# OVGULIU/cedar

Measured on AMD Instinct MI355X. Metric: fine-grid DOF/s per V-cycle, higher is better.
Workload: dtype f64; 1 GPU; 3D 27-pt gallery::fe Poisson-type, 512^3, 8-colour GS V(2,1); levels=8, cycle=V(2,1), relaxation=point, parallelism=single GPU

## Files before the change

cedar_amd/csrc/relax27_dev.h:

```cpp
#pragma once
#include "common.h"

namespace cedar_amd {

struct C27 {
	real_t pw, ps, psw, b, bw, bs, bsw;
	real_t pnw_n, ps_n, bnw_n, bn_n;
	real_t b_t, be_t, bn_t, bne_t;
	real_t bse_nt, bs_nt;
	real_t psw_ne, bne_ne;
	real_t pw_e, pnw_e, be_e, bse_e;
	real_t bsw_net;
	real_t bw_et, bnw_et;
};

__device__ __forceinline__ real_t offdiag27(real_t qf, const C27 &c, const real_t (&qq)[3][3][3])
{
	real_t s = qf;
	s = s + c.pw * qq[1][1][0];
	s = s + c.pnw_n * qq[1][2][0];
	s = s + c.ps_n * qq[1][2][1];
	s = s + c.psw_ne * qq[1][2][2];
	s = s + c.pw_e * qq[1][1][2];
	s = s + c.pnw_e * qq[1][0][2];
	s = s + c.ps * qq[1][0][1];
	s = s + c.psw * qq[1][0][0];
	s = s + c.b * qq[0][1][1];
	s = s + c.bw * qq[0][1][0];
	s = s + c.bnw_n * qq[0][2][0];
	s = s + c.bn_n * qq[0][2][1];
	s = s + c.bne_ne * qq[0][2][2];
	s = s + c.be_e * qq[0][1][2];
	s = s + c.bse_e * qq[0][0][2];
	s = s + c.bs * qq[0][0][1];
	s = s + c.bsw * qq[0][0][0];
	s = s + c.b_t * qq[2][1][1];
	s = s + c.be_t * qq[2][1][0];
	s = s + c.bse_nt * qq[2][2][0];
	s = s + c.bs_nt * qq[2][2][1];
	s = s + c.bsw_net * qq[2][2][2];
	s = s + c.bw_et * qq[2][1][2];
	s = s + c.bnw_et * qq[2][0][2];
	s = s + c.bn_t * qq[2][0][1];
	s = s + c.bne_t * qq[2][0][0];
	return s;
}


__device__ __forceinline__ void ldpair(const real_t *__restrict__ p, bool two, real_t &a, real_t &b)
{
	if (two) {
		d2u v = *reinterpret_cast<const d2u *>(p);
		a = v.x; b = v.y;
	} else {
		a = p[0]; b = 0.0;
	}
}

__device__ __forceinline__ void ldpair(const float *__restrict__ p, bool two, real_t &a, real_t &b)
{
	if (two) {
		f2u v = *reinterpret_cast<const f2u *>(p);
		a = (real_t)v.x; b = (real_t)v.y;
	} else {
		a = (real_t)p[0]; b = 0.0;
	}
}

template <bool NT>
__device__ __forceinline__ void ldpair_so(const real_t *__restrict__ p, bool two, real_t &a, real_t &b)
{
	if (!NT) { ldpair(p, two, a, b); return; }
	if (two) {
		d2u v = __builtin_nontemporal_load(reinterpret_cast<const d2u *>(p));
		a = v.x; b = v.y;
	} else {
		a = __builtin_nontemporal_load(p); b = 0.0;
	}
}

template <bool NT>
__device__ __forceinline__ void ldpair_so(const float *__restrict__ p, bool two, real_t &a, real_t &b)
{
	if (!NT) { ldpair(p, two, a, b); return; }
	if (two) {
		f2u v = __builtin_nontemporal_load(reinterpret_cast<const f2u *>(p));
		a = (real_t)v.x; b = (real_t)v.y;
	} else {
		a = (real_t)__builtin_nontemporal_load(p); b = 0.0;
	}
}

#define WI_SLOT(slot) ((size_t)(((WI & 4) && ((slot) == KB || (slot) >= KBW)) ? KPW : (slot)))
template <bool NT, bool NTP = NT, bool NTO = NT, int WI = 0, typename OP = Op3>
__device__ __forceinline__ void load_coef27(const OP &A, size_t rowA, int ie, int io, bool two, C27 &ce, C27 &co)
{
	const auto *__restrict__ so = A.so;
	const size_t PS = A.SS, aj = A.SJ, ak = (WI & 2) ? 0 : A.SK;
#define LD_I_(N, slot, off, fe, fo)                                                    \
{                                                                                  \
	real_t a_, b_;                                                                 \
	ldpair_so<N>(so + WI_SLOT(slot)*PS + rowA + (off) + ie, true, a_, b_);         \
	ce.fe = a_; co.fo = b_;                                                        \
}
#define LD_I(slot, off, fe, fo) LD_I_(NT, slot, off, fe, fo)
#define LD_IO(slot, fe, fo) LD_I_(NTO, slot, 0, fe, fo)
#define LD_IS(slot, off, fe, fo) LD_I_(NTP, slot, off, fe, fo)
#define LD_ISO(slot, fe, fo) LD_I_((NTP && NTO), slot, 0, fe, fo)
	LD_IO(KPW, pw, pw) LD_ISO(KPS, ps, ps) LD_ISO(KPSW, psw, psw) LD_IO(KB, b, b)
	LD_IO(KBW, bw, bw) LD_IO(KBS, bs, bs) LD_IO(KBSW, bsw, bsw)
	LD_IS(KPNW, aj, pnw_n, pnw_n) LD_IS(KPS, aj, ps_n, ps_n) LD_I(KBNW, aj, bnw_n, bnw_n) LD_I(KBN, aj, bn_n, bn_n)
	LD_I(KB, ak, b_t, b_t) LD_I(KBE, ak, be_t, be_t) LD_I(KBN, ak, bn_t, bn_t) LD_I(KBNE, ak, bne_t, bne_t)
	LD_I(KBSE, aj + ak, bse_nt, bse_nt) LD_I(KBS, aj + ak, bs_nt, bs_nt)
#undef LD_I
#undef LD_IO
#undef LD_IS
#undef LD_ISO
#undef LD_I_
#define LD_IP_(N, slot, off, f)                                                        \
{                                                                                  \
	real_t a_, b_;                                                                 \
	ldpair_so<N>(so + WI_SLOT(slot)*PS + rowA + (off) + io, two, a_, b_);          \
	ce.f = a_; co.f = b_;                                                          \
}
#define LD_IP(slot, off, f) LD_IP_(NT, slot, off, f)
#define LD_IPO(slot, f) LD_IP_(NTO, slot, 0, f)
#define LD_IPS(slot, off, f) LD_IP_(NTP, slot, off, f)
#define LD_IPSO(slot, f) LD_IP_((NTP && NTO), slot, 0, f)
	LD_IPS(KPSW, aj, psw_ne) LD_IP(KBNE, aj, bne_ne)
	LD_IPO(KPW, pw_e) LD_IPSO(KPNW, pnw_e) LD_IPO(KBE, be_e) LD_IPO(KBSE, bse_e)
	LD_IP(KBSW, aj + ak, bsw_net)
	LD_IP(KBW, ak, bw_et) LD_IP(KBNW, ak, bnw_et)
#undef LD_IP
#undef LD_IPO
#undef LD_IPS
#undef LD_IPSO
#undef LD_IP_
}

template <int WI = 0>
__device__ __forceinline__ void load_vec27(const real_t *__restrict__ qf, const real_t *__restrict__ q, size_t row, size_t sj,
                                           size_t sk, int ie, int io, bool two,
                                           real_t (&qe)[3][3][3], real_t (&qo)[3][3][3], real_t &qfe, real_t &qfo)
{
	if (WI & 1) { sj = 0; sk = 0; }
	{
		real_t a_, b_;
		ldpair(qf + row + ie, true, a_, b_); qfe = a_; qfo = b_;
	}
#pragma unroll
	for (int dk = 0; dk < 3; dk++)
#pragma unroll
		for (int dj = 0; dj < 3; dj++) {
			const real_t *r = q + row + (ptrdiff_t)(dj - 1) * (ptrdiff_t)sj + (ptrdiff_t)(dk - 1) * (ptrdiff_t)sk;
			real_t w0, w1, w2, w3;
			ldpair(r + ie - 1, true, w0, w1);
			ldpair(r + io, two, w2, w3);
			qe[dk][dj][0] = w0; qe[dk][dj][1] = w1; qe[dk][dj][2] = w2;
			qo[dk][dj][0] = w1; qo[dk][dj][1] = w2; qo[dk][dj][2] = w3;
		}
}

template <bool NT, bool NTP = NT, bool NTO = NT, int WI = 0, typename OP = Op3>
__device__ __forceinline__ void load_pair27(const OP &A, const real_t *__restrict__ qf,
                                            const real_t *__restrict__ q, size_t rowA, size_t row, size_t sj, size_t sk,
                                            int ie, int io, bool two, C27 &ce, C27 &co,
                                            real_t (&qe)[3][3][3], real_t (&qo)[3][3][3], real_t &qfe, real_t &qfo)
{
	load_coef27<NT, NTP, NTO, WI>(A, rowA, ie, io, two, ce, co);
	load_vec27<WI>(qf, q, row, sj, sk, ie, io, two, qe, qo, qfe, qfo);
}

__device__ __forceinline__ void skip27_lane(unsigned skm, int p, int P, bool &ske, bool &sko)
{
	if (skm & 0x100u) { ske = sko = true; return; }
	const int slot = p == 0 ? 0 : p == 1 ? 2 : p == P - 2 ? 4 : p == P - 1 ? 6 : -1;
	ske = slot >= 0 && ((skm >> slot) & 1u);
	sko = slot >= 0 && ((skm >> (slot + 1)) & 1u);
}

template <int BS, bool EFIRST, bool NT, bool NTP = NT, int WI = 0, bool PERX = false, bool MSK = false, typename OP = Op3>
__device__ __forceinline__ void relax27_row_task(const OP &A, const real_t *__restrict__ qf,
                                                 real_t *__restrict__ q, int II, size_t sj, size_t sk,
                                                 size_t j, size_t k, real_t *xch, unsigned skm = 0)
{
	const size_t row = j * sj + k * sk, rowA = j * A.SJ + k * A.SK;
	const int p = threadIdx.x;
	const int ie = 2 * p + 1, io = 2 * p + 2;
	const bool e_ok = ie <= II - 2;
	const bool o_ok = io <= II - 2;
	const bool two = io + 1 <= II - 1;

	real_t e_new = 0.0, o_new = 0.0;
	C27 ce, co;
	real_t qe[3][3][3], qo[3][3][3];
	real_t qfe = 0, qfo = 0, sre = 0, sro = 0;

	if (e_ok) {
		load_pair27<NT, NTP, NT, WI>(A, qf, q, rowA, row, sj, sk, ie, io, two, ce, co, qe, qo, qfe, qfo);
		real_t a_, b_;
		ldpair(A.sor + j * A.rSJ + k * A.rSK + ie, true, a_, b_); sre = a_; sro = b_;
	}

	bool ske = false, sko = false;
	if (MSK) skip27_lane(skm, p, (II - 2 + 1) / 2, ske, sko);
	if (EFIRST) {
		if (e_ok) {
			e_new = (MSK && ske) ? qe[1][1][1] : offdiag27(qfe, ce, qe) * sre;
			xch[p] = e_new;
		}
		__syncthreads();
		if (o_ok) {
			qo[1][1][0] = e_new;
			if (io + 1 <= II - 2) qo[1][1][2] = xch[p + 1];
			else if (PERX) qo[1][1][2] = xch[0];
			o_new = (MSK && sko) ? qo[1][1][1] : offdiag27(qfo, co, qo) * sro;
		}
		if (PERX && o_ok && io == II - 2) {
			q[row] = o_new;
			q[row + II - 1] = xch[0];
		}
	} else {
		if (o_ok) {
			o_new = (MSK && sko) ? qo[1][1][1] : offdiag27(qfo, co, qo) * sro;
			xch[p + 1] = o_new;
		}
		__syncthreads();
		if (e_ok) {
			if (p > 0) qe[1][1][0] = xch[p];
			else if (PERX) qe[1][1][0] = xch[(II - 2) / 2];
			if (o_ok) qe[1][1][2] = o_new;
			e_new = (MSK && ske) ? qe[1][1][1] : offdiag27(qfe, ce, qe) * sre;
		}
		if (PERX && p == 0 && e_ok) {
			q[row] = xch[(II - 2) / 2];
			q[row + II - 1] = e_new;
		}
	}
	if (e_ok) {
		if (o_ok) {
			d2u v; v.x = e_new; v.y = o_new;
			*reinterpret_cast<d2u *>(q + row + ie) = v;
		} else {
			q[row + ie] = e_new;
		}
	}
}

}
```

cedar_amd/csrc/relax3d_psum.hip:

```cpp
#include "common.h"
#include "relax27_dev.h"
#include "relax3_psum.h"
#include <vector>

namespace cedar_amd {

struct PsumGeom { int jbF, frun, nF, nS, nrun; };

__host__ __device__ static inline PsumGeom psum_geom(int JJ, int jbF, int frun)
{
	PsumGeom g;
	g.jbF = jbF; g.frun = frun;
	g.nF = (JJ - 2 - jbF + 1) / 2;
	g.nS = (JJ - 2 - (1 - jbF) + 1) / 2;
	g.nrun = (g.nF + frun - 1) / frun;
	return g;
}

__host__ __device__ static inline void psum_run_range(const PsumGeom &g, int JJ, int run, int &lo, int &hi)
{
	const int f0 = run * g.frun, f1 = (f0 + g.frun < g.nF) ? f0 + g.frun : g.nF;
	lo = 1 + g.jbF + 2 * f0;
	hi = 1 + g.jbF + 2 * (f1 - 1);
	if (g.jbF && f0 == 0) lo = 1;
	if (f1 == g.nF && hi + 1 <= JJ - 2) hi = hi + 1;
}

__host__ __device__ static inline bool psum_row_ok(const PsumGeom &g, int JJ, int j)
{
	int f = (j - 1 - g.jbF) >> 1;
	if (f < 0) f = 0;
	if (f >= g.nF) f = g.nF - 1;
	int lo, hi;
	psum_run_range(g, JJ, f / g.frun, lo, hi);
	return lo + 1 <= j && j <= hi - 1;
}

__host__ __device__ static inline bool psum_a_gives(int k, int KK, int nbr)
{
	return k >= 1 && k <= KK - 2 && !(k == 1 && (nbr & 1)) && !(k == KK - 2 && (nbr & 2));
}
__host__ __device__ static inline bool psum_b_takes(int kp, int KK, int nbr)
{
	return kp - 1 >= 1 && kp + 1 <= KK - 2 && psum_a_gives(kp - 1, KK, nbr) && psum_a_gives(kp + 1, KK, nbr);
}

template <int SIDE, int DI, int DJ>
__device__ __forceinline__ real_t kcoef(const C27 &c)
{
	if (SIDE == 0) {
		if (DI == 0 && DJ == 0) return c.b_t;
		if (DI == -1 && DJ == 0) return c.be_t;
		if (DI == -1 && DJ == 1) return c.bse_nt;
		if (DI == 0 && DJ == 1) return c.bs_nt;
		if (DI == 1 && DJ == 1) return c.bsw_net;
		if (DI == 1 && DJ == 0) return c.bw_et;
		if (DI == 1 && DJ == -1) return c.bnw_et;
		if (DI == 0 && DJ == -1) return c.bn_t;
		return c.bne_t;
	}
	if (DI == 0 && DJ == 0) return c.b;
	if (DI == -1 && DJ == 0) return c.bw;
	if (DI == -1 && DJ == 1) return c.bnw_n;
	if (DI == 0 && DJ == 1) return c.bn_n;
	if (DI == 1 && DJ == 1) return c.bne_ne;
	if (DI == 1 && DJ == 0) return c.be_e;
	if (DI == 1 && DJ == -1) return c.bse_e;
	if (DI == 0 && DJ == -1) return c.bs;
	return c.bsw;
}

template <int BS>
struct PsumLds {
	real_t xch[2][BS + 2];
	real_t exP[6][BS + 1];
	real_t exN[6][BS + 1];
	real_t acc[4][2][2 * BS];
};

template <int BS, bool EFIRST, bool NT, typename OP = Op3>
__device__ __forceinline__ void relax27_row_task_A(const OP &A, const real_t *__restrict__ qf, real_t *__restrict__ q,
                                                   real_t *__restrict__ T, int II, size_t sj, size_t sk, size_t j, size_t k,
                                                   PsumLds<BS> &S, int t, bool isf, int lo, int hi, bool stU, bool stD,
                                                   unsigned skm)
{
	const size_t row = j * sj + k * sk, rowA = j * A.SJ + k * A.SK;
	const int p = threadIdx.x;
	const int ie = 2 * p + 1, io = 2 * p + 2;
	const bool e_ok = ie <= II - 2;
	const bool o_ok = io <= II - 2;
	const bool two = io + 1 <= II - 1;
	real_t *xch = S.xch[t & 1];

	real_t e_new = 0.0, o_new = 0.0;
	C27 ce, co;
	real_t qe[3][3][3], qo[3][3][3];
	real_t qfe = 0, qfo = 0, sre = 0, sro = 0;

	if (e_ok) {
		load_pair27<NT, false, NT, 0>(A, qf, q, rowA, row, sj, sk, ie, io, two, ce, co, qe, qo, qfe, qfo);
		real_t a_, b_;
		ldpair(A.sor + j * A.rSJ + k * A.rSK + ie, true, a_, b_); sre = a_; sro = b_;
	}
	const real_t ghostL = qe[1][1][0];
	const real_t ghostR = o_ok ? qo[1][1][2] : qe[1][1][2];

	bool ske = false, sko = false;
	if (skm) skip27_lane(skm, p, (II - 2 + 1) / 2, ske, sko);
	if (EFIRST) {
		if (e_ok) {
			e_new = ske ? qe[1][1][1] : offdiag27(qfe, ce, qe) * sre;
			xch[p] = e_new;
		}
		__syncthreads();
		if (o_ok) {
			qo[1][1][0] = e_new;
			if (io + 1 <= II - 2) qo[1][1][2] = xch[p + 1];
			o_new = sko ? qo[1][1][1] : offdiag27(qfo, co, qo) * sro;
		}
	} else {
		if (o_ok) {
			o_new = sko ? qo[1][1][1] : offdiag27(qfo, co, qo) * sro;
			xch[p + 1] = o_new;
		}
		__syncthreads();
		if (e_ok) {
			if (p > 0) qe[1][1][0] = xch[p];
			if (o_ok) qe[1][1][2] = o_new;
			e_new = ske ? qe[1][1][1] : offdiag27(qfe, ce, qe) * sre;
		}
	}
	if (e_ok) {
		if (o_ok) {
			d2u v; v.x = e_new; v.y = o_new;
			*reinterpret_cast<d2u *>(q + row + ie) = v;
		} else {
			q[row + ie] = e_new;
		}
	}
	if (!stU && !stD) return;

	const real_t se = e_new, so_ = o_ok ? o_new : ghostR;
	const bool last_o = o_ok && io == II - 2;
	real_t own_e[6], own_o[6];
	const auto *__restrict__ sop = A.so;
	const size_t PS = A.SS, aj = A.SJ, ak = A.SK;
	if (e_ok) {
#define GROUP(SIDE, DJ)                                                                                           \
	{                                                                                                             \
		constexpr int g_ = SIDE * 3 + (DJ + 1);                                                                   \
		own_e[g_] = se * kcoef<SIDE, 0, DJ>(ce);                                                                  \
		if (o_ok || io == II - 1) own_e[g_] = own_e[g_] + so_ * kcoef<SIDE, -1, DJ>(co);                          \
		S.exP[g_][p] = se * kcoef<SIDE, -1, DJ>(ce);                                                              \
		if (o_ok) {                                                                                               \
			own_o[g_] = se * kcoef<SIDE, 1, DJ>(ce) + so_ * kcoef<SIDE, 0, DJ>(co);                               \
			S.exN[g_][p + 1] = so_ * kcoef<SIDE, 1, DJ>(co);                                                      \
		}                                                                                                         \
	}
		GROUP(0, -1) GROUP(0, 0) GROUP(0, 1) GROUP(1, -1) GROUP(1, 0) GROUP(1, 1)
#undef GROUP
		if (p == 0) {
			S.exN[0][0] = ghostL * sop[KBNW * PS + rowA + ak + 1];
			S.exN[1][0] = ghostL * sop[KBW * PS + rowA + ak + 1];
			S.exN[2][0] = ghostL * sop[KBSW * PS + rowA + aj + ak + 1];
			S.exN[3][0] = ghostL * sop[KBSE * PS + rowA + 1];
			S.exN[4][0] = ghostL * sop[KBE * PS + rowA + 1];
			S.exN[5][0] = ghostL * sop[KBNE * PS + rowA + aj + 1];
		}
		if (last_o) {
			const size_t x = (size_t)(II - 1);
			S.exP[0][p + 1] = ghostR * sop[KBNE * PS + rowA + ak + x];
			S.exP[1][p + 1] = ghostR * sop[KBE * PS + rowA + ak + x];
			S.exP[2][p + 1] = ghostR * sop[KBSE * PS + rowA + aj + ak + x];
			S.exP[3][p + 1] = ghostR * sop[KBSW * PS + rowA + x];
			S.exP[4][p + 1] = ghostR * sop[KBW * PS + rowA + x];
			S.exP[5][p + 1] = ghostR * sop[KBNW * PS + rowA + aj + x];
		}
	}
	__syncthreads();
	if (e_ok) {
#pragma unroll
		for (int g = 0; g < 6; g++) {
			const int side = g / 3, dj = g % 3 - 1;
			real_t *a = S.acc[((int)j + dj) & 3][side] + 2 * p;
			const real_t te = (S.exN[g][p] + own_e[g]);
			const bool add = !isf || dj < 0;
			a[0] = add ? a[0] + te : te;
			if (o_ok) {
				const real_t to = own_o[g] + S.exP[g][p + 1];
				a[1] = add ? a[1] + to : to;
			}
		}
		if (!isf) {
#pragma unroll
			for (int c = 0; c < 2; c++) {
				const int r = (int)j - 1 + c;
				if (r < lo + 1 || r > hi - 1) continue;
#pragma unroll
				for (int side = 0; side < 2; side++) {
					if (side == 0 ? !stU : !stD) continue;
					const real_t *a = S.acc[r & 3][side] + 2 * p;
					real_t *dst = T + (size_t)r * sj + (side == 0 ? k + 1 : k) * sk + ie;
					if (o_ok) {
						d2u v; v.x = a[0]; v.y = a[1];
						*reinterpret_cast<d2u *>(dst) = v;
					} else
						dst[0] = a[0];
				}
			}
		}
	}
}

template <int BS, bool EFIRST, bool NT, typename OP = Op3>
__global__ __launch_bounds__(BS) void relax27_planeA(const OP A, const real_t *__restrict__ qf, real_t *__restrict__ q,
                                                      real_t *__restrict__ T, int II, int JJ, int KK, int kb, int kr0,
                                                      int nrk, int nbr, PsumGeom gm, PsumSkip skp)
{
	__shared__ PsumLds<BS> S;
	const unsigned nblk = (unsigned)nrk * (unsigned)gm.nrun;
	const unsigned L = xcd_remap(blockIdx.x, nblk);
	if (L >= nblk) return;
	const int kr = (int)(L / (unsigned)gm.nrun), run = (int)(L % (unsigned)gm.nrun);
	const int jbF = gm.jbF, nF = gm.nF, nS = gm.nS;
	const int f0 = run * gm.frun, f1 = min(nF, f0 + gm.frun);
	int lo, hi;
	psum_run_range(gm, JJ, run, lo, hi);
	const size_t sj = (size_t)II, sk = (size_t)II * JJ;
	const int ki = 1 + kb + 2 * (kr + kr0);
	const size_t k = (size_t)ki;
	const bool stU = psum_b_takes(ki + 1, KK, nbr), stD = psum_b_takes(ki - 1, KK, nbr);
	int t = 0;
	for (int f = f0; f < f1; f++) {
		relax27_row_task_A<BS, EFIRST, NT>(A, qf, q, T, II, sj, sk, (size_t)(1 + jbF + 2 * f), k, S, t, true, lo, hi, stU, stD,
		                                   psum_skip_mask(skp, 1 + jbF + 2 * f, true));
		t++;
		const int g = jbF ? f : f - 1;
		const bool have = jbF ? (f > f0 || f == 0) : (f > f0);
		if (have && g >= 0 && g < nS) {
			__syncthreads();
			relax27_row_task_A<BS, EFIRST, NT>(A, qf, q, T, II, sj, sk, (size_t)(2 - jbF + 2 * g), k, S, t, false, lo, hi, stU, stD,
			                                   psum_skip_mask(skp, 2 - jbF + 2 * g, false));
			t++;
		}
	}
	if (f1 == nF && f1 > f0) {
		const int g = jbF ? nF : nF - 1;
		if (g < nS) {
			__syncthreads();
			relax27_row_task_A<BS, EFIRST, NT>(A, qf, q, T, II, sj, sk, (size_t)(2 - jbF + 2 * g), k, S, t, false, lo, hi, stU, stD,
			                                   psum_skip_mask(skp, 2 - jbF + 2 * g, false));
			t++;
		}
	}
}

template <int BS, bool EFIRST, bool NT, typename OP = Op3>
__device__ __forceinline__ void relax27_row_task_B(const OP &A, const real_t *__restrict__ qf, real_t *__restrict__ q,
                                                   const real_t *__restrict__ T, int II, size_t sj, size_t sk, size_t j,
                                                   size_t k, real_t *xch, unsigned skm)
{
	const size_t row = j * sj + k * sk, rowA = j * A.SJ + k * A.SK;
	const int p = threadIdx.x;
	const int ie = 2 * p + 1, io = 2 * p + 2;
	const bool e_ok = ie <= II - 2;
	const bool o_ok = io <= II - 2;
	const bool two = io + 1 <= II - 1;
	const auto *__restrict__ so = A.so;
	const size_t PS = A.SS, aj = A.SJ;

	real_t pw_e = 0, pw_o = 0, ps_e = 0, ps_o = 0, psw_e = 0, psw_o = 0, pnwn_e = 0, pnwn_o = 0, psn_e = 0, psn_o = 0;
	real_t pswne_e = 0, pswne_o = 0, pwe_e = 0, pwe_o = 0, pnwe_e = 0, pnwe_o = 0;
	real_t qfe = 0, qfo = 0, sre = 0, sro = 0, tbe = 0, tbo = 0, tte = 0, tto = 0;
	real_t w[3][4];
	if (e_ok) {
		ldpair_so<NT>(so + KPW * PS + rowA + ie, true, pw_e, pw_o);
		ldpair(so + KPS * PS + rowA + ie, true, ps_e, ps_o);
		ldpair(so + KPSW * PS + rowA + ie, true, psw_e, psw_o);
		ldpair(so + KPNW * PS + rowA + aj + ie, true, pnwn_e, pnwn_o);
		ldpair(so + KPS * PS + rowA + aj + ie, true, psn_e, psn_o);
		ldpair(so + KPSW * PS + rowA + aj + io, two, pswne_e, pswne_o);
		ldpair_so<NT>(so + KPW * PS + rowA + io, two, pwe_e, pwe_o);
		ldpair(so + KPNW * PS + rowA + io, two, pnwe_e, pnwe_o);
		ldpair(A.sor + j * A.rSJ + k * A.rSK + ie, true, sre, sro);
		ldpair(qf + row + ie, true, qfe, qfo);
		ldpair_so<NT>(T + row + ie, true, tbe, tbo);
		ldpair_so<NT>(T + row + sk + ie, true, tte, tto);
#pragma unroll
		for (int dj = 0; dj < 3; dj++) {
			const real_t *r = q + row + (ptrdiff_t)(dj - 1) * (ptrdiff_t)sj;
			ldpair(r + ie - 1, true, w[dj][0], w[dj][1]);
			ldpair(r + io, two, w[dj][2], w[dj][3]);
		}
	}
#define INPLANE(qf_, pw_, pnwn_, psn_, pswne_, pwe_, pnwe_, ps_, psw_, W, C, E, tb_, tt_) \
	((((((((((qf_ + pw_ * W(1)) + pnwn_ * W(2)) + psn_ * C(2)) + pswne_ * E(2)) + pwe_ * E(1)) + pnwe_ * E(0)) + ps_ * C(0)) + psw_ * W(0)) + tb_) + tt_)
	real_t e_new = 0.0, o_new = 0.0;
	bool ske = false, sko = false;
	if (skm) skip27_lane(skm, p, (II - 2 + 1) / 2, ske, sko);
	const real_t e_old = w[1][1], o_old = w[1][2];
	if (EFIRST) {
		if (e_ok) {
#define W_(d) w[d][0]
#define C_(d) w[d][1]
#define E_(d) w[d][2]
			e_new = INPLANE(qfe, pw_e, pnwn_e, psn_e, pswne_e, pwe_e, pnwe_e, ps_e, psw_e, W_, C_, E_, tbe, tte) * sre;
#undef W_
#undef C_
#undef E_
			if (ske) e_new = e_old;
			xch[p] = e_new;
		}
		__syncthreads();
		if (o_ok) {
			w[1][1] = e_new;
			if (io + 1 <= II - 2) w[1][3] = xch[p + 1];
#define W_(d) w[d][1]
#define C_(d) w[d][2]
#define E_(d) w[d][3]
			o_new = INPLANE(qfo, pw_o, pnwn_o, psn_o, pswne_o, pwe_o, pnwe_o, ps_o, psw_o, W_, C_, E_, tbo, tto) * sro;
#undef W_
#undef C_
#undef E_
			if (sko) o_new = o_old;
		}
	} else {
		if (o_ok) {
#define W_(d) w[d][1]
#define C_(d) w[d][2]
#define E_(d) w[d][3]
			o_new = INPLANE(qfo, pw_o, pnwn_o, psn_o, pswne_o, pwe_o, pnwe_o, ps_o, psw_o, W_, C_, E_, tbo, tto) * sro;
#undef W_
#undef C_
#undef E_
			if (sko) o_new = o_old;
			xch[p + 1] = o_new;
		}
		__syncthreads();
		if (e_ok) {
			if (p > 0) w[1][0] = xch[p];
			if (o_ok) w[1][2] = o_new;
#define W_(d) w[d][0]
#define C_(d) w[d][1]
#define E_(d) w[d][2]
			e_new = INPLANE(qfe, pw_e, pnwn_e, psn_e, pswne_e, pwe_e, pnwe_e, ps_e, psw_e, W_, C_, E_, tbe, tte) * sre;
#undef W_
#undef C_
#undef E_
			if (ske) e_new = e_old;
		}
	}
#undef INPLANE
	if (e_ok) {
		if (o_ok) {
			d2u v; v.x = e_new; v.y = o_new;
			*reinterpret_cast<d2u *>(q + row + ie) = v;
		} else {
			q[row + ie] = e_new;
		}
	}
}

template <int BS, bool EFIRST, bool NT, typename OP = Op3>
__global__ __launch_bounds__(BS) void relax27_planeB(const OP A, const real_t *__restrict__ qf, real_t *__restrict__ q,
                                                      const real_t *__restrict__ T, int II, int JJ, int KK, int kb, int kr0,
                                                      int nrk, PsumGeom gm, PsumSkip skp)
{
	__shared__ real_t xch[2][BS + 2];
	const unsigned nblk = (unsigned)nrk * (unsigned)gm.nrun;
	const unsigned L = xcd_remap(blockIdx.x, nblk);
	if (L >= nblk) return;
	const int kr = (int)(L / (unsigned)gm.nrun), run = (int)(L % (unsigned)gm.nrun);
	const int jbF = gm.jbF, nF = gm.nF, nS = gm.nS;
	const int f0 = run * gm.frun, f1 = min(nF, f0 + gm.frun);
	int lo, hi;
	psum_run_range(gm, JJ, run, lo, hi);
	const size_t sj = (size_t)II, sk = (size_t)II * JJ;
	const size_t k = (size_t)(1 + kb + 2 * (kr + kr0));
	int t = 0;
	for (int f = f0; f < f1; f++) {
		const int jf = 1 + jbF + 2 * f;
		const unsigned mf = psum_skip_mask(skp, jf, true);
		if (jf >= lo + 1 && jf <= hi - 1 && !(mf & 0x100u)) {
			if (t) __syncthreads();
			relax27_row_task_B<BS, EFIRST, NT>(A, qf, q, T, II, sj, sk, (size_t)jf, k, xch[t & 1], mf);
			t++;
		}
		const int g = jbF ? f : f - 1;
		const bool have = jbF ? (f > f0 || f == 0) : (f > f0);
		const int js = 2 - jbF + 2 * g;
		const unsigned ms = psum_skip_mask(skp, js, false);
		if (have && g >= 0 && g < nS && js >= lo + 1 && js <= hi - 1 && !(ms & 0x100u)) {
			if (t) __syncthreads();
			relax27_row_task_B<BS, EFIRST, NT>(A, qf, q, T, II, sj, sk, (size_t)js, k, xch[t & 1], ms);
			t++;
		}
	}
}

template <int BS, bool EFIRST, bool NT, typename OP = Op3>
__global__ __launch_bounds__(BS) void relax27_rows_sel(const OP A, const real_t *__restrict__ qf, real_t *__restrict__ q,
                                                        int II, int JJ, int KK, int kb, int elo, int ehi, int x0, int x1,
                                                        PsumGeom gm, int cls, PsumSkip skp)
{
	__shared__ real_t xch[BS + 2];
	const int nrows = cls ? gm.nS : gm.nF;
	const int nx = (x0 >= 0 ? 1 : 0) + (x1 >= 0 ? 1 : 0);
	int w = (int)blockIdx.x;
	int kr, j;
	if (w < nx * nrows) {
		const int tpl = w / nrows, r = w % nrows;
		kr = (tpl == 0 && x0 >= 0) ? x0 : x1;
		j = (cls ? 2 - gm.jbF : 1 + gm.jbF) + 2 * r;
	} else {
		w -= nx * nrows;
		const int ncand = cls ? gm.nrun + 1 : 2 * gm.nrun;
		kr = elo + w / ncand;
		const int c = w % ncand;
		if (kr >= ehi) return;
		if (cls == 0) {
			const int run = c >> 1, end = c & 1;
			const int f0 = run * gm.frun, f1 = min(gm.nF, f0 + gm.frun);
			if (end && f1 - 1 == f0) return;
			j = 1 + gm.jbF + 2 * (end ? f1 - 1 : f0);
			if (psum_row_ok(gm, JJ, j)) return;
		} else {
			if (c < gm.nrun - 1) {
				const int f1 = (c + 1) * gm.frun;
				j = 1 + gm.jbF + 2 * f1 - 1;
			} else if (c == gm.nrun - 1) {
				if (!gm.jbF) return;
				j = 1;
			} else {
				j = 1 + gm.jbF + 2 * (gm.nF - 1) + 1;
				if (j > JJ - 2) return;
			}
			if (j < 1 || j > JJ - 2) return;
		}
	}
	const size_t sj = (size_t)II, sk = (size_t)II * JJ;
	const unsigned m = psum_skip_mask(skp, j, cls == 0);
	if (m & 0x100u) return;
	relax27_row_task<BS, EFIRST, NT, NT, 0, false, true>(A, qf, q, II, sj, sk, (size_t)j, (size_t)(1 + kb + 2 * kr), xch, m);
}

template <int BS, bool EFIRST, bool NT, typename OP = Op3>
__global__ __launch_bounds__(BS) void relax27_rows_between(const OP A, const real_t *__restrict__ qf, real_t *__restrict__ q,
                                                            int II, int JJ, int KK, int j0, int jstep, int nrj, int kb, int kr0,
                                                            int nrk, PsumSkip skp)
{
	__shared__ real_t xch[BS + 2];
	const int w = (int)blockIdx.x;
	if (w >= nrj * nrk) return;
	const size_t sj = (size_t)II, sk = (size_t)II * JJ;
	const int j = j0 + jstep * (w % nrj);
	const unsigned m = psum_skip_mask(skp, j, false);
	if (m & 0x100u) return;
	relax27_row_task<BS, EFIRST, NT, NT, 0, false, true>(A, qf, q, II, sj, sk, (size_t)j, (size_t)(1 + kb + 2 * (kr0 + w / nrj)), xch, m);
}

template <int BS, bool EFIRST, typename OP>
static void phase_a(const OP &A, const real_t *qf, real_t *q, real_t *T, int II, int JJ, int KK, int kb, int kr0, int nrk,
                    int nbr, const PsumGeom &gm, hipStream_t st, const PsumSkip &skp)
{
	if (nrk <= 0) return;
	hipLaunchKernelGGL((relax27_planeA<BS, EFIRST, true, OP>), dim3(xcd_grid((unsigned)nrk * (unsigned)gm.nrun)), dim3(BS), 0, st,
	                   A, qf, q, T, II, JJ, KK, kb, kr0, nrk, nbr, gm, skp);
	if (gm.nrun > 1)
		hipLaunchKernelGGL((relax27_rows_between<BS, EFIRST, true, OP>), dim3((unsigned)((gm.nrun - 1) * nrk)), dim3(BS), 0, st,
		                   A, qf, q, II, JJ, KK, (gm.jbF ? 1 : 0) + 2 * gm.frun, 2 * gm.frun, gm.nrun - 1, kb, kr0, nrk, skp);
}

template <int BS, bool EFIRST, typename OP>
static void phase_b(const OP &A, const real_t *qf, real_t *q, real_t *T, int II, int JJ, int KK, int kb, int kr0, int nrk,
                    int nbr, const PsumGeom &gm, hipStream_t st, const PsumSkip &skp)
{
	if (nrk <= 0) return;
	int elo = kr0, ehi = kr0 + nrk, x0 = -1, x1 = -1;
	while (elo < ehi && !psum_b_takes(1 + kb + 2 * elo, KK, nbr)) elo++;
	while (ehi > elo && !psum_b_takes(1 + kb + 2 * (ehi - 1), KK, nbr)) ehi--;
	std::vector<int> exact;
	for (int kr = kr0; kr < kr0 + nrk; kr++)
		if (kr < elo || kr >= ehi) exact.push_back(kr);
	const int nel = ehi - elo;
	size_t done = 0;
	do {
		x0 = done < exact.size() ? exact[done] : -1;
		x1 = done + 1 < exact.size() ? exact[done + 1] : -1;
		const bool first = done == 0;
		done += 2;
		const int nxp = (x0 >= 0 ? 1 : 0) + (x1 >= 0 ? 1 : 0);
		for (int cls = 0; cls < 2; cls++) {
			if (cls == 1 && first && nel > 0)
				hipLaunchKernelGGL((relax27_planeB<BS, EFIRST, true, OP>), dim3(xcd_grid((unsigned)nel * (unsigned)gm.nrun)), dim3(BS), 0, st,
				                   A, qf, q, T, II, JJ, KK, kb, elo, nel, gm, skp);
			const int nrows = cls ? gm.nS : gm.nF, ncand = cls ? gm.nrun + 1 : 2 * gm.nrun;
			const int nwg = nxp * nrows + (first ? nel * ncand : 0);
			if (nwg > 0)
				hipLaunchKernelGGL((relax27_rows_sel<BS, EFIRST, true, OP>), dim3((unsigned)nwg), dim3(BS), 0, st,
				                   A, qf, q, II, JJ, KK, kb, first ? elo : 0, first ? ehi : 0, x0, x1, gm, cls, skp);
		}
	} while (done < exact.size());
}

template <int BS, bool EFIRST, typename OP>
static void sweep_psum(const OP &A, const real_t *qf, real_t *q, real_t *T, int II, int JJ, int KK, int frun, hipStream_t st)
{
	const bool up = EFIRST;
	const int jbF = up ? 0 : 1, kbA = up ? 0 : 1, kbB = 1 - kbA;
	const PsumGeom gm = psum_geom(JJ, jbF, frun);
	const PsumSkip none = psum_skip_none();
	phase_a<BS, EFIRST>(A, qf, q, T, II, JJ, KK, kbA, 0, (KK - 2 - kbA + 1) / 2, 0, gm, st, none);
	phase_b<BS, EFIRST>(A, qf, q, T, II, JJ, KK, kbB, 0, (KK - 2 - kbB + 1) / 2, 0, gm, st, none);
}

void relax3_planes27_psum(const Op3 &A, const real_t *qf, real_t *q, real_t *T, int II, int JJ, int KK, int kb, int up, int kr0,
                          int nrk, int nbr, int frun, hipStream_t st, const PsumSkip *skip)
{
	const int npairs = (II - 2 + 1) / 2;
	const PsumGeom gm = psum_geom(JJ, up ? 0 : 1, frun);
	const PsumSkip skp = skip ? *skip : psum_skip_none();
	const bool first_parity = up ? kb == 0 : kb == 1;
#define PSUM_PH(B)                                                                                                  \
	do {                                                                                                            \
		if (first_parity) {                                                                                         \
			if (up) phase_a<B, true>(A, qf, q, T, II, JJ, KK, kb, kr0, nrk, nbr, gm, st, skp);                          \
			else phase_a<B, false>(A, qf, q, T, II, JJ, KK, kb, kr0, nrk, nbr, gm, st, skp);                            \
		} else {                                                                                                    \
			if (up) phase_b<B, true>(A, qf, q, T, II, JJ, KK, kb, kr0, nrk, nbr, gm, st, skp);                          \
			else phase_b<B, false>(A, qf, q, T, II, JJ, KK, kb, kr0, nrk, nbr, gm, st, skp);                            \
		}                                                                                                           \
	} while (0)
	if (npairs <= 64) PSUM_PH(64);
	else if (npairs <= 128) PSUM_PH(128);
	else PSUM_PH(256);
#undef PSUM_PH
}

bool relax3_psum_ok(int II, int JJ, int KK, int frun)
{
	return frun > 0 && II >= 3 && JJ >= 3 && KK >= 3 && (II - 2 + 1) / 2 <= 256;
}

template <typename OP>
static void relax3_gs27_psum_t(const OP &A, const real_t *qf, real_t *q, real_t *T, int II, int JJ, int KK, int updown, int frun,
                               hipStream_t st)
{
	const int npairs = (II - 2 + 1) / 2;
	const bool up = updown == BMG_UP;
#define PSUM_BS(B)                                                                   \
	do {                                                                             \
		if (up) sweep_psum<B, true>(A, qf, q, T, II, JJ, KK, frun, st);              \
		else sweep_psum<B, false>(A, qf, q, T, II, JJ, KK, frun, st);                \
	} while (0)
	if (npairs <= 64) PSUM_BS(64);
	else if (npairs <= 128) PSUM_BS(128);
	else PSUM_BS(256);
#undef PSUM_BS
}

void relax3_gs27_psum(const Op3 &A, const real_t *qf, real_t *q, real_t *T, int II, int JJ, int KK, int updown, int frun,
                      hipStream_t st)
{
	relax3_gs27_psum_t(A, qf, q, T, II, JJ, KK, updown, frun, st);
}

void relax3_gs27_psum(const Op3f &A, const real_t *qf, real_t *q, real_t *T, int II, int JJ, int KK, int updown, int frun,
                      hipStream_t st)
{
	relax3_gs27_psum_t(A, qf, q, T, II, JJ, KK, updown, frun, st);
}

}
```

Baseline: 5.949 billion DOF/s.

## Carry q-row windows in registers across j-rows in psum plane kernels

Adds a register carry for the 27-point stencil's vector windows so that, as a workgroup walks j-rows within a plane, the k±1 neighbour rows and the shared j-row already loaded by the previous task are reused instead of reloaded from global memory. Phase A reuses both the k-neighbour windows and one in-plane row. Phase B reuses the in-plane row carried from the previous row. The path is on by default for block sizes of at least 128 and can be toggled with an environment variable. It trades fewer global loads for extra registers and branching, which could reduce occupancy or cause spills.

```diff
diff --git a/cedar_amd/csrc/relax27_dev.h b/cedar_amd/csrc/relax27_dev.h
--- a/cedar_amd/csrc/relax27_dev.h
+++ b/cedar_amd/csrc/relax27_dev.h
@@ -161,6 +161,80 @@
 		}
 }
 
+__device__ __forceinline__ void ldwin27(const real_t *__restrict__ r, int ie, int io, bool two, real_t (&w)[4])
+{
+	ldpair(r + ie - 1, true, w[0], w[1]);
+	ldpair(r + io, two, w[2], w[3]);
+}
+
+struct Carry27A {
+	real_t n[2][4][4];
+	real_t c[4];
+	int cb, valid, cj;
+};
+
+__device__ __forceinline__ void carry27_reset(Carry27A &C)
+{
+	C.cb = -8; C.valid = 0; C.cj = -1;
+}
+
+template <bool ISF>
+__device__ __forceinline__ void load_vec27_carry(const real_t *__restrict__ qf, const real_t *__restrict__ q, size_t row, size_t sj,
+                                                 size_t sk, int j, bool e_ok, int ie, int io, bool two, Carry27A &C,
+                                                 real_t (&qe)[3][3][3], real_t (&qo)[3][3][3], real_t &qfe, real_t &qfo)
+{
+	constexpr int S0 = ISF ? 1 : 0;
+	const int nb = j - 1 - S0;
+	if (nb == C.cb + 2) {
+#pragma unroll
+		for (int side = 0; side < 2; side++)
+#pragma unroll
+			for (int x = 0; x < 4; x++) {
+				C.n[side][0][x] = C.n[side][2][x];
+				C.n[side][1][x] = C.n[side][3][x];
+			}
+		C.valid >>= 2;
+	} else if (nb != C.cb) {
+		C.valid = 0;
+	}
+	C.cb = nb;
+	const bool khit = ISF && C.cj == j - 1;
+	real_t wk[3][4];
+	if (e_ok) {
+		real_t a_, b_;
+		ldpair(qf + row + ie, true, a_, b_); qfe = a_; qfo = b_;
+#pragma unroll
+		for (int dj = 0; dj < 3; dj++) {
+			const real_t *r = q + row + (ptrdiff_t)(dj - 1) * (ptrdiff_t)sj;
+#pragma unroll
+			for (int side = 0; side < 2; side++)
+				if (!((C.valid >> (S0 + dj)) & 1)) ldwin27(side ? r + sk : r - sk, ie, io, two, C.n[side][S0 + dj]);
+			if (dj == 0 && khit) {
+#pragma unroll
+				for (int x = 0; x < 4; x++) wk[0][x] = C.c[x];
+			} else {
+				ldwin27(r, ie, io, two, wk[dj]);
+			}
+		}
+	}
+	C.valid |= 7 << S0;
+	if (ISF) {
+#pragma unroll
+		for (int x = 0; x < 4; x++) C.c[x] = wk[2][x];
+		C.cj = j + 1;
+	} else if (C.cj == j) {
+		C.cj = -1;
+	}
+#pragma unroll
+	for (int dk = 0; dk < 3; dk++)
+#pragma unroll
+		for (int dj = 0; dj < 3; dj++) {
+			const real_t (&w)[4] = dk == 1 ? wk[dj] : C.n[dk >> 1][S0 + dj];
+			qe[dk][dj][0] = w[0]; qe[dk][dj][1] = w[1]; qe[dk][dj][2] = w[2];
+			qo[dk][dj][0] = w[1]; qo[dk][dj][1] = w[2]; qo[dk][dj][2] = w[3];
+		}
+}
+
 template <bool NT, bool NTP = NT, bool NTO = NT, int WI = 0, typename OP = Op3>
 __device__ __forceinline__ void load_pair27(const OP &A, const real_t *__restrict__ qf,
                                             const real_t *__restrict__ q, size_t rowA, size_t row, size_t sj, size_t sk,
diff --git a/cedar_amd/csrc/relax3d_psum.hip b/cedar_amd/csrc/relax3d_psum.hip
--- a/cedar_amd/csrc/relax3d_psum.hip
+++ b/cedar_amd/csrc/relax3d_psum.hip
@@ -1,6 +1,8 @@
 #include "common.h"
 #include "relax27_dev.h"
 #include "relax3_psum.h"
+#include <cstdlib>
+#include <type_traits>
 #include <vector>
 
 namespace cedar_amd {
@@ -78,11 +80,11 @@
 	real_t acc[4][2][2 * BS];
 };
 
-template <int BS, bool EFIRST, bool NT, typename OP = Op3>
+template <int BS, bool EFIRST, bool NT, typename OP = Op3, bool CARRY = false>
 __device__ __forceinline__ void relax27_row_task_A(const OP &A, const real_t *__restrict__ qf, real_t *__restrict__ q,
                                                    real_t *__restrict__ T, int II, size_t sj, size_t sk, size_t j, size_t k,
                                                    PsumLds<BS> &S, int t, bool isf, int lo, int hi, bool stU, bool stD,
-                                                   unsigned skm)
+                                                   unsigned skm, Carry27A &CR)
 {
 	const size_t row = j * sj + k * sk, rowA = j * A.SJ + k * A.SK;
 	const int p = threadIdx.x;
@@ -98,9 +100,14 @@
 	real_t qfe = 0, qfo = 0, sre = 0, sro = 0;
 
 	if (e_ok) {
-		load_pair27<NT, false, NT, 0>(A, qf, q, rowA, row, sj, sk, ie, io, two, ce, co, qe, qo, qfe, qfo);
+		if (CARRY) load_coef27<NT, false, NT, 0>(A, rowA, ie, io, two, ce, co);
+		else load_pair27<NT, false, NT, 0>(A, qf, q, rowA, row, sj, sk, ie, io, two, ce, co, qe, qo, qfe, qfo);
 		real_t a_, b_;
 		ldpair(A.sor + j * A.rSJ + k * A.rSK + ie, true, a_, b_); sre = a_; sro = b_;
+	}
+	if (CARRY) {
+		if (isf) load_vec27_carry<true>(qf, q, row, sj, sk, (int)j, e_ok, ie, io, two, CR, qe, qo, qfe, qfo);
+		else load_vec27_carry<false>(qf, q, row, sj, sk, (int)j, e_ok, ie, io, two, CR, qe, qo, qfe, qfo);
 	}
 	const real_t ghostL = qe[1][1][0];
 	const real_t ghostR = o_ok ? qo[1][1][2] : qe[1][1][2];
@@ -212,7 +219,7 @@
 	}
 }
 
-template <int BS, bool EFIRST, bool NT, typename OP = Op3>
+template <int BS, bool EFIRST, bool NT, typename OP = Op3, bool CARRY = false>
 __global__ __launch_bounds__(BS) void relax27_planeA(const OP A, const real_t *__restrict__ qf, real_t *__restrict__ q,
                                                       real_t *__restrict__ T, int II, int JJ, int KK, int kb, int kr0,
                                                       int nrk, int nbr, PsumGeom gm, PsumSkip skp)
@@ -230,17 +237,19 @@
 	const int ki = 1 + kb + 2 * (kr + kr0);
 	const size_t k = (size_t)ki;
 	const bool stU = psum_b_takes(ki + 1, KK, nbr), stD = psum_b_takes(ki - 1, KK, nbr);
+	Carry27A CR;
+	carry27_reset(CR);
 	int t = 0;
 	for (int f = f0; f < f1; f++) {
-		relax27_row_task_A<BS, EFIRST, NT>(A, qf, q, T, II, sj, sk, (size_t)(1 + jbF + 2 * f), k, S, t, true, lo, hi, stU, stD,
-		                                   psum_skip_mask(skp, 1 + jbF + 2 * f, true));
+		relax27_row_task_A<BS, EFIRST, NT, OP, CARRY>(A, qf, q, T, II, sj, sk, (size_t)(1 + jbF + 2 * f), k, S, t, true, lo, hi, stU, stD,
+		                                              psum_skip_mask(skp, 1 + jbF + 2 * f, true), CR);
 		t++;
 		const int g = jbF ? f : f - 1;
 		const bool have = jbF ? (f > f0 || f == 0) : (f > f0);
 		if (have && g >= 0 && g < nS) {
 			__syncthreads();
-			relax27_row_task_A<BS, EFIRST, NT>(A, qf, q, T, II, sj, sk, (size_t)(2 - jbF + 2 * g), k, S, t, false, lo, hi, stU, stD,
-			                                   psum_skip_mask(skp, 2 - jbF + 2 * g, false));
+			relax27_row_task_A<BS, EFIRST, NT, OP, CARRY>(A, qf, q, T, II, sj, sk, (size_t)(2 - jbF + 2 * g), k, S, t, false, lo, hi, stU, stD,
+			                                              psum_skip_mask(skp, 2 - jbF + 2 * g, false), CR);
 			t++;
 		}
 	}
@@ -248,17 +257,17 @@
 		const int g = jbF ? nF : nF - 1;
 		if (g < nS) {
 			__syncthreads();
-			relax27_row_task_A<BS, EFIRST, NT>(A, qf, q, T, II, sj, sk, (size_t)(2 - jbF + 2 * g), k, S, t, false, lo, hi, stU, stD,
-			                                   psum_skip_mask(skp, 2 - jbF + 2 * g, false));
+			relax27_row_task_A<BS, EFIRST, NT, OP, CARRY>(A, qf, q, T, II, sj, sk, (size_t)(2 - jbF + 2 * g), k, S, t, false, lo, hi, stU, stD,
+			                                              psum_skip_mask(skp, 2 - jbF + 2 * g, false), CR);
 			t++;
 		}
 	}
 }
 
-template <int BS, bool EFIRST, bool NT, typename OP = Op3>
+template <int BS, bool EFIRST, bool NT, typename OP = Op3, bool CARRY = false>
 __device__ __forceinline__ void relax27_row_task_B(const OP &A, const real_t *__restrict__ qf, real_t *__restrict__ q,
                                                    const real_t *__restrict__ T, int II, size_t sj, size_t sk, size_t j,
-                                                   size_t k, real_t *xch, unsigned skm)
+                                                   size_t k, real_t *xch, unsigned skm, bool isf, real_t (&cw)[4], int &cj)
 {
 	const size_t row = j * sj + k * sk, rowA = j * A.SJ + k * A.SK;
 	const int p = threadIdx.x;
@@ -273,6 +282,7 @@
 	real_t pswne_e = 0, pswne_o = 0, pwe_e = 0, pwe_o = 0, pnwe_e = 0, pnwe_o = 0;
 	real_t qfe = 0, qfo = 0, sre = 0, sro = 0, tbe = 0, tbo = 0, tte = 0, tto = 0;
 	real_t w[3][4];
+	const bool hit = CARRY && isf && cj == (int)j - 1;
 	if (e_ok) {
 		ldpair_so<NT>(so + KPW * PS + rowA + ie, true, pw_e, pw_o);
 		ldpair(so + KPS * PS + rowA + ie, true, ps_e, ps_o);
@@ -289,8 +299,21 @@
 #pragma unroll
 		for (int dj = 0; dj < 3; dj++) {
 			const real_t *r = q + row + (ptrdiff_t)(dj - 1) * (ptrdiff_t)sj;
-			ldpair(r + ie - 1, true, w[dj][0], w[dj][1]);
-			ldpair(r + io, two, w[dj][2], w[dj][3]);
+			if (dj == 0 && hit) {
+#pragma unroll
+				for (int x = 0; x < 4; x++) w[0][x] = cw[x];
+			} else {
+				ldwin27(r, ie, io, two, w[dj]);
+			}
+		}
+	}
+	if (CARRY) {
+		if (isf) {
+#pragma unroll
+			for (int x = 0; x < 4; x++) cw[x] = w[2][x];
+			cj = (int)j + 1;
+		} else if (cj == (int)j) {
+			cj = -1;
 		}
 	}
 #define INPLANE(qf_, pw_, pnwn_, psn_, pswne_, pwe_, pnwe_, ps_, psw_, W, C, E, tb_, tt_) \
@@ -361,7 +384,7 @@
 	}
 }
 
-template <int BS, bool EFIRST, bool NT, typename OP = Op3>
+template <int BS, bool EFIRST, bool NT, typename OP = Op3, bool CARRY = false>
 __global__ __launch_bounds__(BS) void relax27_planeB(const OP A, const real_t *__restrict__ qf, real_t *__restrict__ q,
                                                       const real_t *__restrict__ T, int II, int JJ, int KK, int kb, int kr0,
                                                       int nrk, PsumGeom gm, PsumSkip skp)
@@ -377,13 +400,15 @@
 	psum_run_range(gm, JJ, run, lo, hi);
 	const size_t sj = (size_t)II, sk = (size_t)II * JJ;
 	const size_t k = (size_t)(1 + kb + 2 * (kr + kr0));
+	real_t cw[4];
+	int cj = -1;
 	int t = 0;
 	for (int f = f0; f < f1; f++) {
 		const int jf = 1 + jbF + 2 * f;
 		const unsigned mf = psum_skip_mask(skp, jf, true);
 		if (jf >= lo + 1 && jf <= hi - 1 && !(mf & 0x100u)) {
 			if (t) __syncthreads();
-			relax27_row_task_B<BS, EFIRST, NT>(A, qf, q, T, II, sj, sk, (size_t)jf, k, xch[t & 1], mf);
+			relax27_row_task_B<BS, EFIRST, NT, OP, CARRY>(A, qf, q, T, II, sj, sk, (size_t)jf, k, xch[t & 1], mf, true, cw, cj);
 			t++;
 		}
 		const int g = jbF ? f : f - 1;
@@ -392,7 +417,7 @@
 		const unsigned ms = psum_skip_mask(skp, js, false);
 		if (have && g >= 0 && g < nS && js >= lo + 1 && js <= hi - 1 && !(ms & 0x100u)) {
 			if (t) __syncthreads();
-			relax27_row_task_B<BS, EFIRST, NT>(A, qf, q, T, II, sj, sk, (size_t)js, k, xch[t & 1], ms);
+			relax27_row_task_B<BS, EFIRST, NT, OP, CARRY>(A, qf, q, T, II, sj, sk, (size_t)js, k, xch[t & 1], ms, false, cw, cj);
 			t++;
 		}
 	}
@@ -459,13 +484,24 @@
 	relax27_row_task<BS, EFIRST, NT, NT, 0, false, true>(A, qf, q, II, sj, sk, (size_t)j, (size_t)(1 + kb + 2 * (kr0 + w / nrj)), xch, m);
 }
 
+static bool psum_carry(int bs)
+{
+	const char *e = getenv("CEDAR_AMD_PSUM_CARRY");
+	if (e) return atoi(e) != 0;
+	return bs >= 128;
+}
+
 template <int BS, bool EFIRST, typename OP>
 static void phase_a(const OP &A, const real_t *qf, real_t *q, real_t *T, int II, int JJ, int KK, int kb, int kr0, int nrk,
                     int nbr, const PsumGeom &gm, hipStream_t st, const PsumSkip &skp)
 {
 	if (nrk <= 0) return;
-	hipLaunchKernelGGL((relax27_planeA<BS, EFIRST, true, OP>), dim3(xcd_grid((unsigned)nrk * (unsigned)gm.nrun)), dim3(BS), 0, st,
-	                   A, qf, q, T, II, JJ, KK, kb, kr0, nrk, nbr, gm, skp);
+	if (psum_carry(BS))
+		hipLaunchKernelGGL((relax27_planeA<BS, EFIRST, true, OP, true>), dim3(xcd_grid((unsigned)nrk * (unsigned)gm.nrun)), dim3(BS), 0, st,
+		                   A, qf, q, T, II, JJ, KK, kb, kr0, nrk, nbr, gm, skp);
+	else
+		hipLaunchKernelGGL((relax27_planeA<BS, EFIRST, true, OP, false>), dim3(xcd_grid((unsigned)nrk * (unsigned)gm.nrun)), dim3(BS), 0, st,
+		                   A, qf, q, T, II, JJ, KK, kb, kr0, nrk, nbr, gm, skp);
 	if (gm.nrun > 1)
 		hipLaunchKernelGGL((relax27_rows_between<BS, EFIRST, true, OP>), dim3((unsigned)((gm.nrun - 1) * nrk)), dim3(BS), 0, st,
 		                   A, qf, q, II, JJ, KK, (gm.jbF ? 1 : 0) + 2 * gm.frun, 2 * gm.frun, gm.nrun - 1, kb, kr0, nrk, skp);
@@ -483,6 +519,8 @@
 	for (int kr = kr0; kr < kr0 + nrk; kr++)
 		if (kr < elo || kr >= ehi) exact.push_back(kr);
 	const int nel = ehi - elo;
+	constexpr bool can_carry = !(EFIRST && std::is_same<OP, Op3f>::value);
+	const bool carry = can_carry && psum_carry(BS);
 	size_t done = 0;
 	do {
 		x0 = done < exact.size() ? exact[done] : -1;
@@ -491,9 +529,14 @@
 		done += 2;
 		const int nxp = (x0 >= 0 ? 1 : 0) + (x1 >= 0 ? 1 : 0);
 		for (int cls = 0; cls < 2; cls++) {
-			if (cls == 1 && first && nel > 0)
-				hipLaunchKernelGGL((relax27_planeB<BS, EFIRST, true, OP>), dim3(xcd_grid((unsigned)nel * (unsigned)gm.nrun)), dim3(BS), 0, st,
-				                   A, qf, q, T, II, JJ, KK, kb, elo, nel, gm, skp);
+			if (cls == 1 && first && nel > 0) {
+				if (carry)
+					hipLaunchKernelGGL((relax27_planeB<BS, EFIRST, true, OP, can_carry>), dim3(xcd_grid((unsigned)nel * (unsigned)gm.nrun)), dim3(BS), 0, st,
+					                   A, qf, q, T, II, JJ, KK, kb, elo, nel, gm, skp);
+				else
+					hipLaunchKernelGGL((relax27_planeB<BS, EFIRST, true, OP, false>), dim3(xcd_grid((unsigned)nel * (unsigned)gm.nrun)), dim3(BS), 0, st,
+					                   A, qf, q, T, II, JJ, KK, kb, elo, nel, gm, skp);
+			}
 			const int nrows = cls ? gm.nS : gm.nF, ncand = cls ? gm.nrun + 1 : 2 * gm.nrun;
 			const int nwg = nxp * nrows + (first ? nel * ncand : 0);
 			if (nwg > 0)
```

New measurement: 5.800 billion DOF/s. -2.5%, worse.
